# DanielLin94144/E2E-ASR-Pytorch

Hardware: AMD Instinct MI355X
Metric: audio frames/sec (fwd+bwd) LibriSpeech-100 joint CTC-att (higher is better)
Workload: dtype bf16; 1 GPU; config/librispeech_asr.yaml (vgg 0, 4xBiLSTM-320, joint CTC-att 0.5), B=16 x T=1200 x D=160 per GPU, L=180, delta+SpecAugment on GPU, fwd+losses+bwd+grad-allreduce+clip+Adadelta, dropout on; global_batch=16, frames_per_utt=1200, parallelism=dp1

## Files before the change

e2e-asr-pytorch_amd/csrc/ctc.hip:

```cpp
#include "common.h"

namespace {

struct CtcP {
    const float* lp;
    const int64_t* tgt;
    const int64_t* in_len;
    const int64_t* tgt_len;
    float* nll;
    float* loss;
    float* grad;
    float* alpha;
    float* beta;
    int B, T, V, L, Smax;
    float gscale;
};

__device__ __forceinline__ float lse2(float a, float b) {
    const float m = fmaxf(a, b);
    if (m == -INFINITY) return -INFINITY;
    return m + __logf(1.f + __expf(-fabsf(a - b)));
}

__device__ __forceinline__ float lse3(float a, float b, float c) {
    const float m = fmaxf(fmaxf(a, b), c);
    if (m == -INFINITY) return -INFINITY;
    const float md = __builtin_amdgcn_fmed3f(a, b, c), mn = fminf(fminf(a, b), c);
    return m + __logf(1.f + __expf(md - m) + __expf(mn - m));
}

constexpr int CTC_FCH = 8;
constexpr size_t CTC_GRAD_LDS = 60 * 1024;

__global__ __launch_bounds__(1024) void ctc_sweep_kernel(CtcP p, int CF) {
    extern __shared__ __attribute__((aligned(16))) unsigned char smem[];
    const int b = blockIdx.x, back = blockIdx.y;
    const int tid = threadIdx.x, NTH = blockDim.x;
    const int V = p.V, T = p.T;
    int tl = (int)p.tgt_len[b];
    tl = max(0, min(tl, p.L));
    const int S = 2 * tl + 1;
    int Tin = (int)p.in_len[b];
    Tin = max(0, min(Tin, T));
    int* ext = reinterpret_cast<int*>(smem);
    float* buf0 = reinterpret_cast<float*>(ext + p.Smax + 2) + 2;
    float* buf1 = buf0 + p.Smax + 6;
    float* s_lp = buf1 + p.Smax + 4;
    const float* lp = p.lp + (long)b * T * V;
    float* lat = (back ? p.beta : p.alpha) + (long)b * T * p.Smax;

    for (int s = tid; s < p.Smax + 2; s += NTH) ext[s] = (s < S && (s & 1)) ? (int)p.tgt[(long)b * p.L + (s >> 1)] : 0;
    for (int s = tid - 2; s < p.Smax + 2; s += NTH) { buf0[s] = -INFINITY; buf1[s] = -INFINITY; }
    __syncthreads();
    if (Tin == 0) {
        if (!back && tid == 0) {
            const float n = (tl == 0) ? 0.f : INFINITY;
            p.nll[b] = n;
        }
        return;
    }
// ... 16 lines not shown
        __syncthreads();
        for (int i = 0; i < nf; ++i) {
            const int t = back ? Tin - 1 - (c0 + i) : c0 + i;
            const float lpe = s_lp[(t - tlo) * V + e];
            float a;
            if (c0 + i == 0) {
                if (!back) a = (s == 0 || s == 1) ? lpe : -INFINITY;
                else       a = (s == S - 1 || s == S - 2) ? lpe : -INFINITY;
            } else {
                const int d1 = back ? 1 : -1;
                if (label) a = lse3(prev[sr], prev[sr + d1], skip ? prev[sr + 2 * d1] : -INFINITY);
                else       a = lse2(prev[sr], prev[sr + d1]);
                a += lpe;
            }
            if (sok) { cur[s] = a; lat[(long)t * p.Smax + s] = a; }
            __syncthreads();
            float* tmp = prev; prev = cur; cur = tmp;
        }
    }
    if (!back && tid == 0) {
        float ll = prev[S - 1];
        if (S > 1) ll = lse2(ll, prev[S - 2]);
        p.nll[b] = -ll;
    }
}

template <int FCH>
__global__ __launch_bounds__(1024) void ctc_grad_kernel(CtcP p) {
    extern __shared__ __attribute__((aligned(16))) unsigned char smem[];
    const int b = blockIdx.y, t0 = blockIdx.x * FCH;
    const int tid = threadIdx.x, NTH = blockDim.x, lane = tid & 63, wave = tid >> 6, nwave = NTH >> 6;
    const int V = p.V, T = p.T;
    int tl = (int)p.tgt_len[b];
    tl = max(0, min(tl, p.L));
    const int S = 2 * tl + 1;
    int Tin = (int)p.in_len[b];
    Tin = max(0, min(Tin, T));
    float* acc = reinterpret_cast<float*>(smem);
    float* blk = acc + FCH * V;
    const float* lp = p.lp + (long)b * T * V;
    float* grad = p.grad + (long)b * T * V;
    for (int i = tid; i < FCH * V; i += NTH) acc[i] = 0.f;
    const int s = tid;
    const bool sok = s < S;
    const int e = (sok && (s & 1)) ? (int)p.tgt[(long)b * p.L + (s >> 1)] : 0;
    const float nll = p.nll[b];
// ... 22 lines not shown
    for (int f = 0; f < FCH; ++f) {
        if (sok && (s & 1) && t0 + f < Tin) atomicAdd(&acc[f * V + e], occ[f]);
        const float bsum = wave_sum((sok && !(s & 1)) ? occ[f] : 0.f);
        if (lane == 0) blk[f * nwave + wave] = bsum;
    }
    __syncthreads();
    for (int i = tid; i < FCH * V; i += NTH) {
        const int f = i / V, v = i - f * V, t = t0 + f;
        if (t >= T) continue;
        float g = 0.f;
        if (t < Tin) {
            float a = acc[i];
            if (v == 0) for (int w = 0; w < nwave; ++w) a += blk[f * nwave + w];
            if (!(nll < INFINITY)) a = NAN;
            g = scale * (expf(lp[(long)t * V + v]) - a);
        }
        grad[(long)t * V + v] = g;
    }
}

}

extern "C" size_t asr_ctc_loss_workspace_bytes(int B, int T, int L) {
    return 2 * (size_t)B * T * (2 * (size_t)L + 1) * sizeof(float);
}

extern "C" int asr_ctc_loss(const float* logp, const int64_t* targets, const int64_t* input_len, const int64_t* target_len,
                            float* nll, float* loss, float* grad, int B, int T, int V, int L, float gscale,
                            void* workspace, size_t workspace_bytes, asr_stream_t stream) {
    ASR_REQUIRE(logp && targets && input_len && target_len && nll && loss && grad && workspace, ASR_E_ARG, "asr_ctc_loss: null pointer");
    ASR_REQUIRE(B > 0 && T > 0 && V > 1 && L > 0, ASR_E_ARG, "asr_ctc_loss: bad dims");
    ASR_REQUIRE(workspace_bytes >= asr_ctc_loss_workspace_bytes(B, T, L), ASR_E_ARG, "asr_ctc_loss: workspace too small");
    const int Smax = 2 * L + 1;
    float* wsf = (float*)workspace;
    CtcP p{logp, targets, input_len, target_len, nll, loss, grad, wsf, wsf + (size_t)B * T * Smax, B, T, V, L, Smax, gscale};
    ASR_REQUIRE(Smax <= 1024, ASR_E_UNSUPPORTED, "asr_ctc_loss: 2L+1=%d states exceed one workgroup", Smax);
    const int nthr = 64 * ((L + 1 + 63) / 64 + (L + 63) / 64);
    const size_t fixed = (size_t)(Smax + 2) * 4 + 2 * (size_t)(Smax + 6) * 4 + 16;
    int CF = (int)((60 * 1024 - fixed) / ((size_t)V * 4));
    ASR_REQUIRE(CF >= 1, ASR_E_UNSUPPORTED, "asr_ctc_loss: V=%d classes exceed the LDS budget: at most V=%d with 2L+1=%d states "
                "(one frame of log-probs beside the lattice buffers in 60 KB)", V, (int)((60 * 1024 - fixed) / 4), Smax);
    if (CF > T) CF = T;
    const size_t lds_s = fixed + (size_t)CF * V * 4;
    const size_t lds_g1 = (size_t)(V + nthr / 64) * 4;
    ASR_REQUIRE(lds_g1 <= CTC_GRAD_LDS, ASR_E_UNSUPPORTED, "asr_ctc_loss: V=%d classes exceed the %zu bytes of LDS of the gradient kernel",
                V, CTC_GRAD_LDS);
    int fch = CTC_FCH;
    while ((size_t)fch * lds_g1 > CTC_GRAD_LDS) fch >>= 1;
    hipStream_t st = (hipStream_t)stream;
    hipLaunchKernelGGL(ctc_sweep_kernel, dim3(B, 2), dim3(nthr), lds_s, st, p, CF);
    const dim3 gg(cdiv(T, fch), B);
    switch (fch) {
        case 8: hipLaunchKernelGGL(ctc_grad_kernel<8>, gg, dim3(nthr), 8 * lds_g1, st, p); break;
        case 4: hipLaunchKernelGGL(ctc_grad_kernel<4>, gg, dim3(nthr), 4 * lds_g1, st, p); break;
        case 2: hipLaunchKernelGGL(ctc_grad_kernel<2>, gg, dim3(nthr), 2 * lds_g1, st, p); break;
        default: hipLaunchKernelGGL(ctc_grad_kernel<1>, gg, dim3(nthr), lds_g1, st, p); break;
    }
    ASR_LAUNCH_CHECK("asr_ctc_loss");
    return ASR_OK;
}
```

e2e-asr-pytorch_amd/csrc/decoder_persist.hip:

```cpp
#include "decoder_plan.h"

static int g_persist_fwd = -1, g_persist_bwd = -1;
static int g_stream_fwd = -1, g_stream_bwd = -1;
extern "C" int asr_att_decoder_set_persistent(int flags) {
    const int old = (g_persist_fwd != 0 ? 1 : 0) | (g_persist_bwd != 0 ? 2 : 0) | (g_stream_fwd > 0 ? 4 : 0) | (g_stream_bwd > 0 ? 8 : 0);
    g_persist_fwd = flags & 1; g_persist_bwd = (flags >> 1) & 1; g_stream_fwd = (flags >> 2) & 1; g_stream_bwd = (flags >> 3) & 1;
    return old;
}
static void read_switches() {
    if (g_persist_fwd < 0) g_persist_fwd = env_switch("ASR_DEC_PERSIST", 1);
    if (g_persist_bwd < 0) g_persist_bwd = env_switch("ASR_DEC_PERSIST_BWD", 1);
    if (g_stream_fwd < 0) g_stream_fwd = env_switch("ASR_DEC_STREAM", 0);
    if (g_stream_bwd < 0) g_stream_bwd = env_switch("ASR_DEC_STREAM", 0);
}
static FwdPlan fwd_plan(const asr_dec_dims_t& d) { read_switches(); return chosen_plan(persist_plan(d), stream_plan_f(d), g_stream_fwd); }
static BwdPlan bwd_plan(const asr_dec_dims_t& d) { read_switches(); return chosen_plan(persist_plan_b(d), stream_plan_b(d), g_stream_bwd); }

DecPlanInfo dec_fwd_plan_info(const asr_dec_dims_t& d) {
    read_switches();
    const FwdPlan r = persist_plan(d), s = stream_plan_f(d);
    return {chosen_plan(r, s, g_stream_fwd).kind, 0, 0, std::max(r.total, s.total)};
}
DecPlanInfo dec_bwd_plan_info(const asr_dec_dims_t& d) {
    read_switches();
    const BwdPlan r = persist_plan_b(d), s = stream_plan_b(d), pl = chosen_plan(r, s, g_stream_bwd);
    return {pl.kind, pl.NT, std::max(r.NT, s.NT), std::max(r.total, s.total)};
}
float* dec_bwd_dgates(const asr_dec_dims_t& d, void* work) { return bwd_work(d, bwd_plan(d), work).dgates; }

namespace {

size_t dec_fwd_persist_lds(int TE, int NT, int A, int E, int Ks, int KCP, int UPW, int SG2) {
    const int EPL = 16 * cdiv(TE, 16);
    const ConvGeo cg = conv_geo(EPL, Ks);
    const size_t shorts = (size_t)((TE * A + 7) & ~7)
                        + ((TE * E + 7) & ~7)
                        + EPL * FCVX_LD
                        + 8 * cg.IMG_LD
                        + 32 * cg.WKP;
    const size_t floats = (size_t)2 * KCP
                        + ((A + 3) & ~3)
                        + ((A + 3) & ~3)
                        + ((NT * TE + 2 * Ks + 8 + 3) & ~3)
                        + NCW * EPL
                        + ((4 * UPW + 3) & ~3)
                        + (size_t)NT * 2 * SG2;
    return 2 * shorts + 4 * floats;
}

// ... 948 lines not shown
```

e2e-asr-pytorch_amd/src/asr.py:

```python
import math

import torch
import torch.nn as nn

from src import functions as F_hip
from src import hipabi as H
from src.module import RNNLayer, Downsampler, LocationAwareAttention, LSTMParams
from src.util import init_weights_, init_gate_

ALIGN = 64


class _RunCtx(object):

    def __init__(self, model):
        self.anchor = model._anchor
        self.prec = model.prec
        self._model = model

    def next_seed(self):
        self._model._drop_counter += 1
        return (self._model.seed * 1000003 + self._model._drop_counter) & 0xFFFFFFFFFFFF


# ... 210 lines not shown
        msg = ['Model spec.| Encoder\'s downsampling rate of time axis is {}.'.format(self.encoder.sample_rate)]
        if self.encoder.vgg == 1:
            msg.append('           | VGG Extractor w/ time downsampling rate = 4 in encoder enabled.')
        if self.encoder.vgg == 5:
            msg.append('           | VGG Extractor w/ Layer normalization and downsampling rate = 4.')
        if self.enable_ctc:
            msg.append('           | CTC training on encoder enabled ( lambda = {}).'.format(self.ctc_weight))
        if self.enable_att:
            msg.append('           | {} attention decoder enabled ( lambda = {}).'.format(self.attention.mode, 1 - self.ctc_weight))
        msg.append('           | HIP path (gfx950), contraction precision = {}.'.format('bf16' if self.prec == H.BF16 else 'fp32'))
        return msg

    def forward(self, audio_feature, feature_len, decode_step, tf_rate=0.0, teacher=None,
                emb_decoder=None, get_dec_state=False, get_logit=False, ctc_async=False):
        if not audio_feature.is_cuda:
            raise RuntimeError('ASR (HIP path) needs CUDA tensors; there is no CPU fallback')
        if emb_decoder is not None:
            raise NotImplementedError('embedding-regulariser plugin is outside the HIP path')
        ctx = _RunCtx(self)
        feature_len = feature_len.to(audio_feature.device)
        ctc_output, att_output, att_seq, dec_state = None, None, None, None
        encode_feature, encode_len = self.encoder(audio_feature.float(), feature_len, ctx)
        encode_feature = F_hip.to_f32_fn(encode_feature)
        side_ctc = (self.enable_ctc and self.enable_att and self.training and torch.is_grad_enabled() and H.overlap_enabled()
                    and H.ctc_side_enabled() and getattr(self, '_dp', None) is None)
        if self.enable_ctc:
            self.ctc_layer[0]._asr_defer = getattr(self, '_dp', None) is None or H.overlap_dp_enabled()
            if side_ctc:
                with H.side_branch(True, encode_feature, encode_len):
                    ctc_output = F_hip.CTCHeadFn.apply(ctx.anchor, encode_feature, self.ctc_layer[0], self.prec, get_logit)
                ctc_output._asr_side = bool(ctc_async)
            else:
                ctc_output = F_hip.CTCHeadFn.apply(ctx.anchor, encode_feature, self.ctc_layer[0], self.prec, get_logit)
        if self.enable_att:
            L = int(decode_step)
            if not (self.decoder.fast and self.attention.fast and self.emb_drop == 0.0):
                from src.variants import variant_decoder
                att_output, att_seq, hs = variant_decoder(self, ctx.anchor, encode_feature, encode_len, L, teacher,
                                                          float(tf_rate) if teacher is not None else 1.0, ctx)
                if get_dec_state:
                    dec_state = hs
                if side_ctc and not ctc_async:
                    H.join_branch(ctc_output)
                return ctc_output, encode_len, att_output, att_seq, dec_state
            att_output, att_seq, hs = F_hip.AttDecoderFn.apply(ctx.anchor, encode_feature, encode_len, teacher, L, self, self.prec,
                                                               float(tf_rate) if teacher is not None else 1.0)
            if get_dec_state:
                dec_state = hs[:, :, -1, :]
        if side_ctc and not ctc_async:
            H.join_branch(ctc_output)
        return ctc_output, encode_len, att_output, att_seq, dec_state

    def fix_ctc_layer(self):
        for param in self.ctc_layer.parameters():
# ... 2 lines not shown
```

e2e-asr-pytorch_amd/src/functions.py:

```python
import contextlib
import ctypes
import weakref

import torch

from src import hipabi as H


def _empty(shape, like):
    return torch.empty(shape, dtype=torch.float32, device=like.device)


def out_frames(layer, T):
    r = layer.sample_rate
    if r == 1:
        return T, 1
    return ((T + r - 1) // r, 1) if layer.sample_style == 'drop' else (T // r, r)


def lstm_rec(layer, gates, B, T, prec, dy=None, c=None):
    Hd, ND = layer.dim, layer.nd
    nbytes = H.lib().asr_lstm_workspace_bytes(B, Hd, ND)
    ws = H.handoff_acquire(nbytes, gates.device)
    tail = (B, T, Hd, ND, prec, H.ptr(ws), nbytes, H.stream_ptr())
# ... 413 lines not shown
            H.call('asr_loss_mix', H.ptr(g), H.ptr(sv[1]), None, None, H.ptr(gb), H.stream_ptr())
        return ga, None, gb, None


class CTCLossFn(torch.autograd.Function):
    @staticmethod
    def forward(ctx, logp_btv, targets, input_len, target_len):
        logp = logp_btv.contiguous()
        B, T, V = logp.shape
        targets = targets.contiguous()
        L = targets.shape[1]
        if 2 * L + 1 > 1024:
            L = max(1, int(target_len.max()))
            targets = targets[:, :L].contiguous()
        dev = logp.device
        nll = torch.empty(B, dtype=torch.float32, device=dev)
        loss = torch.empty((), dtype=torch.float32, device=dev)
        grad = _empty((B, T, V), logp)
        nbytes = H.lib().asr_ctc_loss_workspace_bytes(B, T, L)
        ws = torch.empty(nbytes, dtype=torch.uint8, device=dev)
        targets = targets.to(dev, torch.int64)
        il = input_len.to(dev, torch.int64).contiguous()
        tl = target_len.to(dev, torch.int64).contiguous()
        H.call('asr_ctc_loss', H.ptr(logp), H.ptr(targets), H.ptr(il), H.ptr(tl), H.ptr(nll), H.ptr(loss), H.ptr(grad),
               B, T, V, L, 1.0, H.ptr(ws), nbytes, H.stream_ptr())
        ctx.save_for_backward(grad)
        ctx.nll = nll
        return loss

    @staticmethod
    def backward(ctx, gout):
        (grad,) = ctx.saved_tensors
        return scale_by_device_scalar(grad, gout), None, None, None


class SeqLossFn(torch.autograd.Function):
    @staticmethod
    def forward(ctx, logits_rv, target_r, mode, classes, smoothing):
        logits = logits_rv.contiguous()
        R, V = logits.shape
        tgt = target_r.to(logits_rv.device, torch.int64).contiguous()
        dev = logits.device
        dl = _empty((R, V), logits)
        loss = torch.empty((), dtype=torch.float32, device=dev)
        acc = torch.empty(4, dtype=torch.float32, device=dev)
        H.call('asr_xent', H.ptr(logits), H.ptr(tgt), R, H.ptr(dl), H.ptr(loss), H.ptr(acc), 1, R, V, mode, classes,
               smoothing, 1.0, H.stream_ptr())
        ctx.save_for_backward(dl)
# ... 233 lines not shown
```

e2e-asr-pytorch_amd/src/hipabi.py:

```python
import atexit
import ctypes
import os

import torch

_HERE = os.path.dirname(os.path.abspath(__file__))
LIB_PATH = os.environ.get('ASR_HIP_LIB') or os.path.join(os.path.dirname(_HERE), 'lib', 'libasr_hip.so')

F32, BF16 = 0, 1
DEBUG_KEEP = os.environ.get('ASR_DEBUG_KEEP', '0') == '1'
ACT_NONE, ACT_TANH, ACT_RELU = 0, 1, 2
MAX_DEC_LAYERS = 4

_vp, _i, _l, _f, _u64, _sz = ctypes.c_void_p, ctypes.c_int, ctypes.c_long, ctypes.c_float, ctypes.c_uint64, ctypes.c_size_t


class DecDims(ctypes.Structure):
    _fields_ = [(n, _i) for n in ('B', 'Tp', 'E', 'A', 'Q', 'Dd', 'NL', 'V', 'Kn', 'Ks', 'L')] + [('temperature', _f)]


_DEC_W_FIELDS = ['Wq', 'bq', 'Wk', 'bk', 'Wconv', 'Wproj', 'wg', 'bg', 'emb']


class DecWeights(ctypes.Structure):
    _fields_ = [(n, _vp) for n in _DEC_W_FIELDS] + \
               [(n, _vp * MAX_DEC_LAYERS) for n in ('Wih', 'Whh', 'bih', 'bhh')] + [('Wc', _vp), ('bc', _vp)]


class DecState(ctypes.Structure):
    _fields_ = ([(n, _vp) for n in ('key', 'att', 'q', 'xin', 'gates', 'cs', 'hs', 'logits', 'energy', 'conv', 'key16', 'enc16', 'work')]
                + [('work_bytes', ctypes.c_size_t), ('tokens', _vp)])


class BeamStep(ctypes.Structure):
    _fields_ = ([(n, _vp) for n in ('att_logp', 'lm_logp', 'psi', 'candidates', 'alive_in', 'sum_in', 'ctcp_in', 'len_in', 'seq_in', 'score_in',
                                    'alive_out', 'sum_out', 'ctcp_out', 'len_out', 'seq_out', 'score_out', 'last_token', 'parent', 'ctc_index',
                                    'tokens')]
                + [('tokens_ld', _l)]
                + [(n, _vp) for n in ('min_len', 'max_len', 'done', 'fin_n', 'fin_len', 'fin_avg', 'fin_seq', 'fin_score')]
                + [(n, _i) for n in ('U', 'beam', 'V', 'C', 'Lmax', 't')]
                + [(n, _f) for n in ('ctc_weight', 'lm_weight', 'eos_threshold')])


ATT_DOT, ATT_LOC = 0, 1
BEAM_ATTEND_MAX_ROWS, BEAM_ATTEND_MAX_T = 16, 8192
CTC_BEAM_MAX = 16


class BeamAttend(ctypes.Structure):
    _fields_ = ([(n, _vp) for n in ('key', 'value', 'q', 'loc', 'wg', 'bg', 'enc_len', 'attn')] + [('attn_ld', _l), ('ctx', _vp)]
                + [(n, _l) for n in ('ctx_ld', 'ld_k', 'ld_v', 'ld_l')]
                + [(n, _i) for n in ('U', 'rows_per_utt', 'NH', 'NHv', 'Tp', 'A', 'Dv', 'mode', 'kv_bf16')] + [('temperature', _f)])


_P = ctypes.POINTER

SIGNATURES = {
    'asr_gemm': [_vp, _vp, _vp, _vp, _i, _i, _i, _l, _l, _l, _i, _i, _i, _i, _i, _i, _l, _l, _l, _i, _i, _i, _vp],
    'asr_lstm_fwd': [_vp, _vp, _vp, _vp, _vp, _i, _i, _i, _i, _i, _vp, _sz, _vp],
    'asr_lstm_bwd': [_vp, _vp, _vp, _vp, _i, _i, _i, _i, _i, _vp, _sz, _vp],
    'asr_dropout_downsample_fwd': [_vp, _vp, _i, _i, _i, _i, _i, _i, _f, _u64, _vp],
    'asr_dropout_downsample_bwd': [_vp, _vp, _i, _i, _i, _i, _i, _i, _f, _u64, _vp],
    'asr_dropout_mask': [_vp, _l, _f, _u64, _vp],
    'asr_act_bwd': [_vp, _vp, _vp, _l, _i, _vp],
    'asr_colsum': [_vp, _l, _i, _i, _vp, _vp],
    'asr_colsum2': [_vp, _l, _i, _i, _vp, _vp, _vp],
    'asr_log_softmax': [_vp, _vp, _l, _i, _vp],
    'asr_logsoftmax_relu_bwd': [_vp, _vp, _vp, _vp, _l, _i, _vp],
    'asr_layernorm_fwd': [_vp, _vp, _vp, _vp, _vp, _l, _i, _f, _i, _vp],
    'asr_layernorm_bwd': [_vp, _vp, _vp, _vp, _vp, _vp, _vp, _vp, _l, _i, _i, _vp],
    'asr_ctc_loss': [_vp, _vp, _vp, _vp, _vp, _vp, _vp, _i, _i, _i, _i, _f, _vp, _sz, _vp],
    'asr_xent': [_vp, _vp, _l, _vp, _vp, _vp, _i, _i, _i, _i, _i, _f, _f, _vp],
    'asr_att_decoder_fwd': [_P(DecDims), _P(DecWeights), _vp, _vp, _vp, _i, _P(DecState), _i, _vp],
    'asr_att_decoder_bwd': [_P(DecDims), _P(DecWeights), _P(DecWeights), _vp, _vp, _P(DecState), _vp, _vp, _vp, _sz, _i, _vp],
    'asr_att_decoder_bwd_ex': [_P(DecDims), _P(DecWeights), _P(DecWeights), _vp, _vp, _P(DecState), _vp, _vp, _vp, _sz, _i, _i,
                               ctypes.POINTER(_i), _vp],
    'asr_att_decoder_bwd_params': [_P(DecDims), _P(DecWeights), _P(DecWeights), _vp, _vp, _P(DecState), _vp, _vp, _sz, _i, _i, _vp],
    'asr_fbank': [_vp, _vp, _vp, _vp, _vp, _vp, _i, _i, _i, _i, _i, _i, _i, _f, _f, _f, _vp, _sz, _vp],
    'asr_delta_stack': [_vp, _vp, _vp, _vp, _i, _i, _i, _i, _i, _vp],
    'asr_specaug': [_vp, _vp, _vp, _vp, _i, _i, _i, _i, _i, _u64, _vp],
    'asr_specaug_ws': [_vp, _vp, _vp, _vp, _i, _i, _i, _i, _i, _u64, _vp, _sz, _vp],
    'asr_conv3x3': [_vp, _vp, _vp, _vp, _i, _i, _i, _i, _i, _i, _i, _i, _i, _vp],
    'asr_conv_weight_permute': [_vp, _vp, _i, _i, _i, _vp],
    'asr_vgg16_im2col': [_vp, _vp, _i, _i, _i, _i, _i, _vp],
    'asr_conv_weight_pack16': [_vp, _vp, _i, _i, _i, _i, _vp],
    'asr_conv_weight_fold': [_vp, _vp, _i, _i, _i, _vp],
    'asr_conv3x3_16': [_vp, _vp, _vp, _vp, _i, _i, _i, _i, _i, _i, _i, _i, _i, _vp],
    'asr_conv3x3_16_wgrad': [_vp, _vp, _vp, _i, _i, _i, _i, _i, _i, _i, _vp],
    'asr_maxpool2x2_16_fwd': [_vp, _vp, _vp, _i, _i, _i, _i, _i, _i, _vp],
    'asr_maxpool2x2_16_bwd': [_vp, _vp, _vp, _i, _i, _i, _i, _i, _i, _vp],
    'asr_ln_freq16_fwd': [_vp, _vp, _vp, _vp, _vp, _i, _i, _i, _i, _f, _i, _vp],
    'asr_ln_freq16_bwd': [_vp, _vp, _vp, _vp, _vp, _vp, _vp, _vp, _vp, _i, _i, _i, _i, _i, _vp],
    'asr_vgg16_output': [_vp, _vp, _i, _i, _i, _i, _vp],
    'asr_vgg16_output_bwd': [_vp, _vp, _i, _i, _i, _i, _vp],
# ... 47 lines not shown
    'asr_cast_bf16': [_vp, _vp, _l, _vp],
    'asr_cast_f32': [_vp, _vp, _l, _i, _vp],
    'asr_rnn_pack_weights': [_vp, _vp, _vp, _vp, _vp, _vp, _vp, _vp, _vp, _i, _i, _i, _i, _vp],
    'asr_dropout_downsample16_fwd': [_vp, _l, _l, _vp, _i, _i, _i, _i, _i, _i, _f, _u64, _vp],
    'asr_dropout_downsample16_bwd': [_vp, _vp, _i, _i, _i, _i, _i, _i, _f, _u64, _vp],
    'asr_act_bwd16': [_vp, _vp, _vp, _l, _i, _vp],
    'asr_colsum16': [_vp, _l, _i, _i, _vp, _vp, _i, _vp],
    'asr_debug_occupy': [_i, _i, ctypes.c_double, _vp],
    'asr_scrub_workspace': [_vp, _sz, _vp, _vp],
    'asr_stream_create_cu_mask': [_i, _i, ctypes.POINTER(_vp)],
    'asr_stream_destroy': [_vp],
}
_RESTYPES = {
    'asr_last_error': (ctypes.c_char_p, []),
    'asr_device_arch': (ctypes.c_char_p, []),
    'asr_version': (ctypes.c_int, []),
    'asr_lstm_workspace_bytes': (_sz, [_i, _i, _i]),
    'asr_gru_rec_workspace_bytes': (_sz, [_i, _i]),
    'asr_specaug_workspace_bytes': (_sz, [_i]),
    'asr_lstm_set_persistent': (ctypes.c_int, [_i]),
    'asr_lstm_plan': (ctypes.c_int, [_i, _i, _i, _i, _i]),
    'asr_lstm16_workspace_bytes': (_sz, [_i, _i, _i, _i]),
    'asr_ctc_loss_workspace_bytes': (_sz, [_i, _i, _i]),
    'asr_ctc_beam_search_workspace_bytes': (_sz, [_i, _i, _i]),
    'asr_ctc_align_workspace_bytes': (_sz, [_i, _i, _i]),
    'asr_fbank_workspace_bytes': (_sz, [_i, _i, _i, _i]),
    'asr_att_decoder_bwd_workspace_bytes': (_sz, [_P(DecDims)]),
    'asr_att_decoder_fwd_work_bytes': (_sz, [_P(DecDims)]),
    'asr_att_decoder_set_persistent': (ctypes.c_int, [_i]),
    'asr_att_decoder_bwd_status_offset': (_sz, [_P(DecDims)]),
    'asr_att_decoder_bwd_persistent_tiles': (ctypes.c_int, [_P(DecDims)]),
    'asr_att_decoder_fwd_plan': (ctypes.c_int, [_P(DecDims)]),
    'asr_att_decoder_bwd_plan': (ctypes.c_int, [_P(DecDims)]),
    'asr_beam_attend_resident_max_t': (ctypes.c_int, [_i]),
}


class HipLibraryMissing(RuntimeError):
    pass


def _load():
    if not os.path.exists(LIB_PATH):
        raise HipLibraryMissing(
            'libasr_hip.so not found at %s — build it with `python -c "import __graft_entry__ as g; g.build()"` '
            '(there is no CPU fallback for the HIP path)' % LIB_PATH)
    lib = ctypes.CDLL(LIB_PATH)
    for name, argtypes in SIGNATURES.items():
        fn = getattr(lib, name)
        fn.argtypes = argtypes
        fn.restype = ctypes.c_int
    for name, (rt, at) in _RESTYPES.items():
        fn = getattr(lib, name)
        fn.argtypes = at
        fn.restype = rt
    return lib
# ... 121 lines not shown


def configure_rec_units(hidden_dims):
    global REC_UNITS
    if 'ASR_REC_UNITS' in os.environ or not hidden_dims:
        return REC_UNITS
    units = max(rec_units_for(h) for h in hidden_dims)
    if units != REC_UNITS:
        if _side['stream'] is not None or _masked:
            release_streams()
        REC_UNITS = units
    return REC_UNITS


def overlap_enabled():
    return os.environ.get('ASR_OVERLAP', '1') != '0'


def overlap_dp_enabled():
    return overlap_enabled() and os.environ.get('ASR_OVERLAP_DP', '0') == '1'


def ctc_side_enabled():
    return os.environ.get('ASR_CTC_SIDE', '0') == '1'


_work = {}


def work_stream():
    dev = torch.cuda.current_device()
    if dev not in _work:
        _work[dev] = torch.cuda.Stream()
    return _work[dev]


def masked_stream(first, count):
    key = (torch.cuda.current_device(), first, count)
    if key not in _masked:
        out = _vp()
        call('asr_stream_create_cu_mask', first, count, ctypes.byref(out))
        _masked[key] = (torch.cuda.ExternalStream(out.value), out.value)
    return _masked[key][0]


def release_streams():
    if not _masked:
# ... 67 lines not shown


class side_branch:

    def __init__(self, wait, *tensors):
        self.wait, self.tensors = wait, [t for t in tensors if t is not None]

    def __enter__(self):
        if _side['stream'] is None:
            _side['stream'] = masked_stream(REC_UNITS, 32 - REC_UNITS) if overlap_enabled() else torch.cuda.Stream()
        side = _side['stream']
        if self.wait:
            side.wait_stream(torch.cuda.current_stream())
        _side['keep'].extend(self.tensors)
        self.ctx = torch.cuda.stream(side)
        self.ctx.__enter__()
        return side

    def __exit__(self, *exc):
        _side['pending'] = True
        return self.ctx.__exit__(*exc)


def join_branch(*tensors):
    cur = torch.cuda.current_stream()
    if _side['stream'] is not None:
        cur.wait_stream(_side['stream'])
    _side['keep'].extend(t for t in tensors if t is not None)


def defer_side(fn, *tensors):
    ev = torch.cuda.Event()
    ev.record(torch.cuda.current_stream())
    _side['deferred'].append((fn, ev, tensors))
    _side['pending'] = True
    if not _side.get('callback'):
        try:
            torch.autograd.Variable._execution_engine.queue_callback(join_side)
            _side['callback'] = True
        except RuntimeError:
            pass


def begin_forward():
    if _side['deferred'] or _side.get('callback'):
        _side['deferred'] = []
        _side['callback'] = False
        del _side['keep'][:]


def flush_side(after=None):
    todo, _side['deferred'] = _side['deferred'], []
    for fn, ev, tensors in todo:
        with on_side_stream(ev, *tensors) as side:
            if after is not None:
                side.wait_event(after)
            fn()


def join_side():
    todo, _side['deferred'] = _side['deferred'], []
    cur = torch.cuda.current_stream()
    for fn, ev, tensors in todo:
        cur.wait_event(ev)
        fn()
    if _side['stream'] is not None and _side['pending']:
        torch.cuda.current_stream().wait_stream(_side['stream'])
    _side['pending'] = False
    _side['callback'] = False
    del _side['keep'][:]
# ... 93 lines not shown
```

e2e-asr-pytorch_amd/src/step.py:

```python
import torch


def train_step(model, optimizer, ctc_crit, att_crit, feat, feat_len, txt, decode_step, tf_rate=1.0, dp=None,
               clip=5.0, txt_len=None, optimize=True):
    from src import hipabi as H
    cur = torch.cuda.current_stream()
    if not (feat.is_cuda and H.overlap_enabled() and (dp is None or H.overlap_dp_enabled())) or cur != torch.cuda.default_stream():
        return _train_step(model, optimizer, ctc_crit, att_crit, feat, feat_len, txt, decode_step, tf_rate, dp, clip, txt_len, optimize)
    work = H.work_stream()
    work.wait_stream(cur)
    with torch.cuda.stream(work):
        out = _train_step(model, optimizer, ctc_crit, att_crit, feat, feat_len, txt, decode_step, tf_rate, dp, clip, txt_len, optimize)
    cur.wait_stream(work)
    for v in out.values():
        if torch.is_tensor(v):
            v.record_stream(cur)
    return out


def scale_weight(w_dev, k):
    from src import hipabi as H
    from src.functions import loss_weight
    if not torch.is_tensor(w_dev):
        return loss_weight(float(w_dev) * k, torch.device('cuda', torch.cuda.current_device()))
    w = w_dev.reshape(1).to(torch.float32).contiguous()
    out = torch.empty(1, dtype=torch.float32, device=w.device)
    H.call('asr_loss_mix', H.ptr(w), H.ptr(loss_weight(k, w.device)), None, None, H.ptr(out), H.stream_ptr())
    return out


def _train_step(model, optimizer, ctc_crit, att_crit, feat, feat_len, txt, decode_step, tf_rate=1.0, dp=None,
                clip=5.0, txt_len=None, optimize=True):
    from src import hipabi as H
    opt = optimizer.opt if hasattr(optimizer, 'opt') else optimizer
    opt.zero_grad()
    if txt_len is None:
        txt_len = torch.sum(txt != 0, dim=-1)
    ctc_output, encode_len, att_output, att_align, _ = model(feat, feat_len, decode_step, tf_rate=tf_rate, teacher=txt, ctc_async=True)
    total, ctc_loss, att_loss = None, None, None
    from src.functions import LossMixFn, loss_weight
    dev = feat.device
    if ctc_output is not None:
        if getattr(ctc_output, '_asr_side', False):
            with H.side_branch(False, txt, txt_len):
                ctc_loss = ctc_crit(ctc_output.transpose(0, 1), txt, encode_len, txt_len)
            H.join_branch(ctc_loss, ctc_output)
        else:
            ctc_loss = ctc_crit(ctc_output.transpose(0, 1), txt, encode_len, txt_len)
    w_att = None
    if att_output is not None:
        b, t, _ = att_output.shape
        att_loss = att_crit(att_output.view(b * t, -1), txt[:, :t].reshape(-1))
        if dp is not None and dp.world > 1:
            w_att = scale_weight(dp.ce_weight(txt_len.sum()), 1 - model.ctc_weight)
        else:
            w_att = loss_weight(1 - model.ctc_weight, dev)
    if ctc_loss is not None and att_loss is not None:
        total = LossMixFn.apply(ctc_loss, loss_weight(model.ctc_weight, dev), att_loss, w_att)
    elif ctc_loss is not None:
        total = LossMixFn.apply(ctc_loss, loss_weight(model.ctc_weight, dev), None, None)
    else:
        total = LossMixFn.apply(att_loss, w_att, None, None)
    total.backward()
    H.join_side()
    grad_mul = 1.0
    if dp is not None:
        dp.finish()
        grad_mul = dp.grad_mul
    normsq = opt.grad_norm()
    if optimize:
        opt.step(clip=clip, grad_mul=grad_mul, use_norm=True)
    return {'total_loss': total.detach(), 'ctc_loss': ctc_loss, 'att_loss': att_loss, 'grad_normsq': normsq,
            'grad_mul': grad_mul, 'ctc_output': ctc_output, 'att_output': att_output, 'att_align': att_align,
            'encode_len': encode_len}
```

include/asr_hip.h:

```cpp
#ifndef ASR_HIP_H
#define ASR_HIP_H
#include <stdint.h>
#include <stddef.h>

#ifdef __cplusplus
extern "C" {
#endif

#define ASR_OK 0
#define ASR_E_ARG (-1)
#define ASR_E_LAUNCH (-2)
#define ASR_E_UNSUPPORTED (-3)

#define ASR_F32 0
#define ASR_BF16 1

#define ASR_ACT_NONE 0
#define ASR_ACT_TANH 1
#define ASR_ACT_RELU 2

typedef void* asr_stream_t;

const char* asr_last_error(void);
int asr_version(void);
// ... 43 lines not shown

int asr_ragged_align(const void* src, void* dst, const int64_t* lens, int B, int T, int ND, int W, int elem_bytes,
                     asr_stream_t stream);
int asr_ragged_unalign(const void* src, long src_bstride, long src_off, void* dst, const int64_t* lens, int B, int T,
                       int ND, int H, int T2, int rate, int style, int elem_bytes, asr_stream_t stream);
int asr_ragged_zero_tail(void* buf, const int64_t* lens, int B, int T, int Ttot, int t_off, int W, int elem_bytes,
                         asr_stream_t stream);

int asr_act_bwd(const float* dout, const float* out, float* dpre, long n, int act, asr_stream_t stream);
int asr_colsum(const float* A, long lda, int M, int N, float* out, asr_stream_t stream);
int asr_colsum2(const float* A, long lda, int M, int N, float* out, float* out2, asr_stream_t stream);
int asr_log_softmax(const float* x, float* out, long rows, int V, asr_stream_t stream);
int asr_logsoftmax_relu_bwd(const float* dlogp, const float* logp, const float* act, float* dpre,
                            long rows, int V, asr_stream_t stream);
int asr_layernorm_fwd(const float* x, const float* w, const float* b, float* y, float* stats,
                      long rows, int n, float eps, int relu, asr_stream_t stream);
int asr_layernorm_bwd(const float* dy, const float* x, const float* w, const float* b, const float* stats,
                      float* dx, float* dw, float* db, long rows, int n, int relu, asr_stream_t stream);

size_t asr_ctc_loss_workspace_bytes(int B, int T, int L);
int asr_ctc_loss(const float* logp, const int64_t* targets, const int64_t* input_len, const int64_t* target_len,
                 float* nll, float* loss, float* grad, int B, int T, int V, int L, float gscale,
                 void* workspace, size_t workspace_bytes, asr_stream_t stream);

int asr_xent(const float* logits, const int64_t* targets, long target_ld, float* dlogits, float* loss,
             float* accum2, int B, int L, int V, int mode, int classes, float smoothing, float gscale,
             asr_stream_t stream);

#define ASR_MAX_DEC_LAYERS 4
typedef struct {
    int B, Tp, E;
    int A, Q;
    int Dd, NL, V;
    int Kn, Ks;
    int L;
    float temperature;
} asr_dec_dims_t;

typedef struct {
    const float *Wq, *bq;
    const float *Wk, *bk;
    const float *Wconv;
    const float *Wproj;
    const float *wg, *bg;
    const float *emb;
    const float *Wih[ASR_MAX_DEC_LAYERS], *Whh[ASR_MAX_DEC_LAYERS];
// ... 11 lines not shown
    float* key;
    float* att;
    float* q;
    float* xin;
    float* gates;
    float* cs;
    float* hs;
    float* logits;
    float* energy;
    float* conv;
    void* key16;
    void* enc16;
    void* work;
    size_t work_bytes;
    int64_t* tokens;
} asr_dec_state_t;

int asr_att_decoder_fwd(const asr_dec_dims_t* dims, const asr_dec_weights_t* weights,
                        const float* enc, const int64_t* enc_len, const int64_t* teacher, int teacher_ld,
                        const asr_dec_state_t* state, int prec, asr_stream_t stream);
size_t asr_att_decoder_bwd_workspace_bytes(const asr_dec_dims_t* dims);
int asr_att_decoder_set_persistent(int flags);
int asr_att_decoder_fwd_plan(const asr_dec_dims_t* dims);
int asr_att_decoder_bwd_plan(const asr_dec_dims_t* dims);
int asr_att_decoder_bwd_persistent_tiles(const asr_dec_dims_t* dims);
size_t asr_att_decoder_bwd_status_offset(const asr_dec_dims_t* dims);
size_t asr_att_decoder_fwd_work_bytes(const asr_dec_dims_t* dims);
int asr_att_decoder_bwd(const asr_dec_dims_t* dims, const asr_dec_weights_t* weights, const asr_dec_grads_t* grads,
                        const float* enc, const int64_t* enc_len, const asr_dec_state_t* state,
                        const float* dlogits, float* denc,
                        void* workspace, size_t workspace_bytes, int prec, asr_stream_t stream);

int asr_att_decoder_bwd_ex(const asr_dec_dims_t* dims, const asr_dec_weights_t* weights, const asr_dec_grads_t* grads,
                           const float* enc, const int64_t* enc_len, const asr_dec_state_t* state,
                           const float* dlogits, float* denc,
                           void* workspace, size_t workspace_bytes, int prec, int defer_params, int* looped_out,
                           asr_stream_t stream);
int asr_att_decoder_bwd_params(const asr_dec_dims_t* dims, const asr_dec_weights_t* weights, const asr_dec_grads_t* grads,
                               const float* enc, const int64_t* enc_len, const asr_dec_state_t* state, const float* dlogits,
                               void* workspace, size_t workspace_bytes, int looped, int prec, asr_stream_t stream);

int asr_sumsq(const float* x, long n, double* out, asr_stream_t stream);
int asr_scale(float* x, long n, float k, asr_stream_t stream);
int asr_scale_dev(const float* in, float* out, long n, const float* alpha, asr_stream_t stream);
int asr_loss_mix(const float* a, const float* wa, const float* b, const float* wb, float* out, asr_stream_t stream);
int asr_status_collect(const void* const* abort_words, int n, unsigned* status, asr_stream_t stream);
// ... 150 lines not shown
```

Baseline: 1.138 million frames/s.

## Run CTC loss on a side stream beside the persistent decoder by default

Turns on the side-stream CTC branch by default. It adds a merged CTC sweep kernel that runs the forward and backward sweeps in one workgroup, claims utterances through global atomics and steers them by XCD. The merged kernel and the gradient kernel pad their LDS request so they can only fit on CUs that the persistent attention decoder leaves free, which lets CTC overlap the decoder without taking its resources. In exchange it adds a header memset, atomic work-claiming, an extra stream wait, and a new path that depends on the fit conditions.

Measured after the change: 1.145 million frames/s (median of 6 runs). About the same (+0.5%).

```diff
diff --git a/e2e-asr-pytorch_amd/csrc/ctc.hip b/e2e-asr-pytorch_amd/csrc/ctc.hip
--- a/e2e-asr-pytorch_amd/csrc/ctc.hip
+++ b/e2e-asr-pytorch_amd/csrc/ctc.hip
@@ -1,4 +1,5 @@
 #include "common.h"
+#include <algorithm>
 
 namespace {
 
@@ -32,10 +33,8 @@
 constexpr int CTC_FCH = 8;
 constexpr size_t CTC_GRAD_LDS = 60 * 1024;
 
-__global__ __launch_bounds__(1024) void ctc_sweep_kernel(CtcP p, int CF) {
-    extern __shared__ __attribute__((aligned(16))) unsigned char smem[];
-    const int b = blockIdx.x, back = blockIdx.y;
-    const int tid = threadIdx.x, NTH = blockDim.x;
+__device__ __forceinline__ void ctc_sweep_utt(const CtcP& p, const int CF, const int b, const int back, const int tid, const int NTH,
+                                              unsigned char* smem) {
     const int V = p.V, T = p.T;
     int tl = (int)p.tgt_len[b];
     tl = max(0, min(tl, p.L));
@@ -98,6 +97,61 @@
         float ll = prev[S - 1];
         if (S > 1) ll = lse2(ll, prev[S - 2]);
         p.nll[b] = -ll;
+    }
+}
+
+__global__ __launch_bounds__(1024) void ctc_sweep_kernel(CtcP p, int CF) {
+    extern __shared__ __attribute__((aligned(16))) unsigned char smem[];
+    ctc_sweep_utt(p, CF, blockIdx.x, blockIdx.y, threadIdx.x, blockDim.x, smem);
+}
+
+constexpr int CTC_W_XCD = 0;
+constexpr int CTC_W_NEXT = 8;
+constexpr int CTC_W_ARRIVED = 9;
+constexpr int CTC_W_UTT = 16;
+inline size_t ctc_hdr_bytes(int B) { return (size_t)(CTC_W_UTT + 2 * B) * sizeof(unsigned); }
+
+__global__ __launch_bounds__(1024) void ctc_sweep_merged_kernel(CtcP p, int CF, unsigned* hdr, int half_bytes) {
+    extern __shared__ __attribute__((aligned(16))) unsigned char smem[];
+    __shared__ int s_b, s_stay;
+    const int NTH = blockDim.x >> 1;
+    const int back = (int)threadIdx.x >= NTH ? 1 : 0;
+    const int tid = threadIdx.x - back * NTH;
+    unsigned char* mine = smem + (size_t)back * half_bytes;
+    unsigned* claim = hdr + CTC_W_UTT;
+    unsigned* done = claim + p.B;
+    if (threadIdx.x == 0) {
+        const unsigned xcc = __builtin_amdgcn_s_getreg((3 << 11) | 20) & 7u;
+        const unsigned ticket = __hip_atomic_fetch_add(&hdr[CTC_W_XCD + xcc], 1u, __ATOMIC_RELAXED, __HIP_MEMORY_SCOPE_AGENT);
+        int b = -1;
+        const unsigned cand = xcc + 8u * ticket;
+        if (ticket < (unsigned)((p.B + 7) >> 3) && cand < (unsigned)p.B &&
+            __hip_atomic_exchange(&claim[cand], 1u, __ATOMIC_RELAXED, __HIP_MEMORY_SCOPE_AGENT) == 0u) b = (int)cand;
+        const unsigned arrived = __hip_atomic_fetch_add(&hdr[CTC_W_ARRIVED], 1u, __ATOMIC_ACQ_REL, __HIP_MEMORY_SCOPE_AGENT);
+        s_b = b;
+        s_stay = (b >= 0 || arrived + 1u == gridDim.x) ? 1 : 0;
+    }
+    __syncthreads();
+    if (!s_stay) return;
+    int b = s_b;
+    while (true) {
+        if (b >= 0) {
+            ctc_sweep_utt(p, CF, b, back, tid, NTH, mine);
+            if (threadIdx.x == 0) __hip_atomic_fetch_add(&done[b], 1u, __ATOMIC_RELAXED, __HIP_MEMORY_SCOPE_AGENT);
+        }
+        __syncthreads();
+        if (threadIdx.x == 0) {
+            int nb = -1;
+            while (true) {
+                const unsigned n = __hip_atomic_fetch_add(&hdr[CTC_W_NEXT], 1u, __ATOMIC_RELAXED, __HIP_MEMORY_SCOPE_AGENT);
+                if (n >= (unsigned)p.B) break;
+                if (__hip_atomic_exchange(&claim[n], 1u, __ATOMIC_RELAXED, __HIP_MEMORY_SCOPE_AGENT) == 0u) { nb = (int)n; break; }
+            }
+            s_b = nb;
+        }
+        __syncthreads();
+        b = s_b;
+        if (b < 0) return;
     }
 }
 
@@ -166,12 +220,28 @@
 }
 
 extern "C" size_t asr_ctc_loss_workspace_bytes(int B, int T, int L) {
-    return 2 * (size_t)B * T * (2 * (size_t)L + 1) * sizeof(float);
+    return 2 * (size_t)B * T * (2 * (size_t)L + 1) * sizeof(float) + ctc_hdr_bytes(B);
+}
+
+static int ctc_sweep_threads(int L) { return 64 * ((L + 1 + 63) / 64 + (L + 63) / 64); }
+
+extern "C" int asr_ctc_loss_merged_threads(int L) {
+    if (L < 1) return 0;
+    const int n = 2 * ctc_sweep_threads(L);
+    return n <= 1024 ? n : 0;
 }
 
 extern "C" int asr_ctc_loss(const float* logp, const int64_t* targets, const int64_t* input_len, const int64_t* target_len,
                             float* nll, float* loss, float* grad, int B, int T, int V, int L, float gscale,
                             void* workspace, size_t workspace_bytes, asr_stream_t stream) {
+    return asr_ctc_loss_ex(logp, targets, input_len, target_len, nll, loss, grad, B, T, V, L, gscale, workspace, workspace_bytes,
+                           ASR_CTC_SPLIT, 0, stream);
+}
+
+extern "C" int asr_ctc_loss_ex(const float* logp, const int64_t* targets, const int64_t* input_len, const int64_t* target_len,
+                               float* nll, float* loss, float* grad, int B, int T, int V, int L, float gscale,
+                               void* workspace, size_t workspace_bytes, int form, size_t min_lds, asr_stream_t stream) {
+    ASR_REQUIRE(form == ASR_CTC_SPLIT || form == ASR_CTC_MERGED || form == ASR_CTC_MERGED_MIN_GRID, ASR_E_ARG, "asr_ctc_loss: form %d", form);
     ASR_REQUIRE(logp && targets && input_len && target_len && nll && loss && grad && workspace, ASR_E_ARG, "asr_ctc_loss: null pointer");
     ASR_REQUIRE(B > 0 && T > 0 && V > 1 && L > 0, ASR_E_ARG, "asr_ctc_loss: bad dims");
     ASR_REQUIRE(workspace_bytes >= asr_ctc_loss_workspace_bytes(B, T, L), ASR_E_ARG, "asr_ctc_loss: workspace too small");
@@ -179,7 +249,7 @@
     float* wsf = (float*)workspace;
     CtcP p{logp, targets, input_len, target_len, nll, loss, grad, wsf, wsf + (size_t)B * T * Smax, B, T, V, L, Smax, gscale};
     ASR_REQUIRE(Smax <= 1024, ASR_E_UNSUPPORTED, "asr_ctc_loss: 2L+1=%d states exceed one workgroup", Smax);
-    const int nthr = 64 * ((L + 1 + 63) / 64 + (L + 63) / 64);
+    const int nthr = ctc_sweep_threads(L);
     const size_t fixed = (size_t)(Smax + 2) * 4 + 2 * (size_t)(Smax + 6) * 4 + 16;
     int CF = (int)((60 * 1024 - fixed) / ((size_t)V * 4));
     ASR_REQUIRE(CF >= 1, ASR_E_UNSUPPORTED, "asr_ctc_loss: V=%d classes exceed the LDS budget: at most V=%d with 2L+1=%d states "
@@ -192,13 +262,32 @@
     int fch = CTC_FCH;
     while ((size_t)fch * lds_g1 > CTC_GRAD_LDS) fch >>= 1;
     hipStream_t st = (hipStream_t)stream;
-    hipLaunchKernelGGL(ctc_sweep_kernel, dim3(B, 2), dim3(nthr), lds_s, st, p, CF);
+    if (form != ASR_CTC_SPLIT && asr_ctc_loss_merged_threads(L)) {
+        constexpr size_t LDS_CAP = 160 * 1024 - 2048;
+        const size_t half = (lds_s + 15) & ~(size_t)15;
+        const size_t lds_m = std::max(2 * half, min_lds);
+        ASR_REQUIRE(lds_m <= LDS_CAP, ASR_E_UNSUPPORTED, "asr_ctc_loss: the merged sweep would need %zu bytes of LDS (limit %zu)", lds_m, LDS_CAP);
+        static unsigned char attr_[32];
+        if (first_on_device(attr_)) hipFuncSetAttribute((const void*)ctc_sweep_merged_kernel, hipFuncAttributeMaxDynamicSharedMemorySize, (int)LDS_CAP);
+        unsigned* hdr = (unsigned*)(wsf + 2 * (size_t)B * T * Smax);
+        hipMemsetAsync(hdr, 0, ctc_hdr_bytes(B), st);
+        const int grid = form == ASR_CTC_MERGED_MIN_GRID ? 1 : 8 * (cdiv(B, 8) + 6);
+        hipLaunchKernelGGL(ctc_sweep_merged_kernel, dim3(grid), dim3(2 * nthr), lds_m, st, p, CF, hdr, (int)half);
+    } else {
+        ASR_REQUIRE(min_lds == 0, ASR_E_UNSUPPORTED, "asr_ctc_loss: L=%d has no merged sweep to run beside other workgroups", L);
+        hipLaunchKernelGGL(ctc_sweep_kernel, dim3(B, 2), dim3(nthr), lds_s, st, p, CF);
+    }
     const dim3 gg(cdiv(T, fch), B);
+    auto launch_grad = [&](auto kernel, int frames) {
+        const size_t lds_g = std::max((size_t)frames * lds_g1, min_lds);
+        if (lds_g > 64 * 1024) hipFuncSetAttribute((const void*)kernel, hipFuncAttributeMaxDynamicSharedMemorySize, (int)(160 * 1024 - 2048));
+        hipLaunchKernelGGL(kernel, gg, dim3(nthr), lds_g, st, p);
+    };
     switch (fch) {
-        case 8: hipLaunchKernelGGL(ctc_grad_kernel<8>, gg, dim3(nthr), 8 * lds_g1, st, p); break;
-        case 4: hipLaunchKernelGGL(ctc_grad_kernel<4>, gg, dim3(nthr), 4 * lds_g1, st, p); break;
-        case 2: hipLaunchKernelGGL(ctc_grad_kernel<2>, gg, dim3(nthr), 2 * lds_g1, st, p); break;
-        default: hipLaunchKernelGGL(ctc_grad_kernel<1>, gg, dim3(nthr), lds_g1, st, p); break;
+        case 8: launch_grad(ctc_grad_kernel<8>, 8); break;
+        case 4: launch_grad(ctc_grad_kernel<4>, 4); break;
+        case 2: launch_grad(ctc_grad_kernel<2>, 2); break;
+        default: launch_grad(ctc_grad_kernel<1>, 1); break;
     }
     ASR_LAUNCH_CHECK("asr_ctc_loss");
     return ASR_OK;
diff --git a/e2e-asr-pytorch_amd/csrc/decoder_persist.hip b/e2e-asr-pytorch_amd/csrc/decoder_persist.hip
--- a/e2e-asr-pytorch_amd/csrc/decoder_persist.hip
+++ b/e2e-asr-pytorch_amd/csrc/decoder_persist.hip
@@ -25,6 +25,16 @@
     read_switches();
     const BwdPlan r = persist_plan_b(d), s = stream_plan_b(d), pl = chosen_plan(r, s, g_stream_bwd);
     return {pl.kind, pl.NT, std::max(r.NT, s.NT), std::max(r.total, s.total)};
+}
+extern "C" size_t asr_att_decoder_ctc_side_lds(const asr_dec_dims_t* dims) {
+    if (!dims) return 0;
+    read_switches();
+    if (!g_persist_fwd) return 0;
+    const FwdPlan pl = fwd_plan(*dims);
+    const int cpx = cdiv(dims->B, 8);
+    if (pl.kind != 1 || dims->B > 16 || 32 - cpx * pl.NT < cpx) return 0;
+    const size_t cu_lds = 160 * 1024, need = cu_lds - std::min(cu_lds, pl.lds) + 2048;
+    return need <= cu_lds - 2048 ? need : 0;
 }
 float* dec_bwd_dgates(const asr_dec_dims_t& d, void* work) { return bwd_work(d, bwd_plan(d), work).dgates; }
 
diff --git a/e2e-asr-pytorch_amd/src/asr.py b/e2e-asr-pytorch_amd/src/asr.py
--- a/e2e-asr-pytorch_amd/src/asr.py
+++ b/e2e-asr-pytorch_amd/src/asr.py
@@ -256,14 +256,20 @@
         ctc_output, att_output, att_seq, dec_state = None, None, None, None
         encode_feature, encode_len = self.encoder(audio_feature.float(), feature_len, ctx)
         encode_feature = F_hip.to_f32_fn(encode_feature)
-        side_ctc = (self.enable_ctc and self.enable_att and self.training and torch.is_grad_enabled() and H.overlap_enabled()
-                    and H.ctc_side_enabled() and getattr(self, '_dp', None) is None)
+        side_lds = 0
+        if (ctc_async and self.enable_ctc and self.enable_att and self.training and torch.is_grad_enabled() and H.overlap_enabled()
+                and getattr(self, '_dp', None) is None and self.prec == H.BF16 and teacher is not None and float(tf_rate) == 1.0
+                and self.decoder.fast and self.attention.fast and self.emb_drop == 0.0):
+            side_lds = H.ctc_side_plan(F_hip._dec_dims(self, encode_feature.shape[0], encode_feature.shape[1], int(decode_step)),
+                                       teacher.shape[1])
+        side_ctc = side_lds > 0
+        self.ctc_side_taken = side_ctc
         if self.enable_ctc:
             self.ctc_layer[0]._asr_defer = getattr(self, '_dp', None) is None or H.overlap_dp_enabled()
             if side_ctc:
                 with H.side_branch(True, encode_feature, encode_len):
                     ctc_output = F_hip.CTCHeadFn.apply(ctx.anchor, encode_feature, self.ctc_layer[0], self.prec, get_logit)
-                ctc_output._asr_side = bool(ctc_async)
+                ctc_output._asr_side = side_lds
             else:
                 ctc_output = F_hip.CTCHeadFn.apply(ctx.anchor, encode_feature, self.ctc_layer[0], self.prec, get_logit)
         if self.enable_att:
diff --git a/e2e-asr-pytorch_amd/src/functions.py b/e2e-asr-pytorch_amd/src/functions.py
--- a/e2e-asr-pytorch_amd/src/functions.py
+++ b/e2e-asr-pytorch_amd/src/functions.py
@@ -459,8 +459,9 @@
         targets = targets.to(dev, torch.int64)
         il = input_len.to(dev, torch.int64).contiguous()
         tl = target_len.to(dev, torch.int64).contiguous()
-        H.call('asr_ctc_loss', H.ptr(logp), H.ptr(targets), H.ptr(il), H.ptr(tl), H.ptr(nll), H.ptr(loss), H.ptr(grad),
-               B, T, V, L, 1.0, H.ptr(ws), nbytes, H.stream_ptr())
+        form = H._ctc_form
+        H.call('asr_ctc_loss_ex', H.ptr(logp), H.ptr(targets), H.ptr(il), H.ptr(tl), H.ptr(nll), H.ptr(loss), H.ptr(grad),
+               B, T, V, L, 1.0, H.ptr(ws), nbytes, form['form'], form['min_lds'], H.stream_ptr())
         ctx.save_for_backward(grad)
         ctx.nll = nll
         return loss
diff --git a/e2e-asr-pytorch_amd/src/hipabi.py b/e2e-asr-pytorch_amd/src/hipabi.py
--- a/e2e-asr-pytorch_amd/src/hipabi.py
+++ b/e2e-asr-pytorch_amd/src/hipabi.py
@@ -44,6 +44,7 @@
 
 ATT_DOT, ATT_LOC = 0, 1
 BEAM_ATTEND_MAX_ROWS, BEAM_ATTEND_MAX_T = 16, 8192
+CTC_SPLIT, CTC_MERGED, CTC_MERGED_MIN_GRID = 0, 1, 2
 CTC_BEAM_MAX = 16
 
 
@@ -70,6 +71,7 @@
     'asr_layernorm_fwd': [_vp, _vp, _vp, _vp, _vp, _l, _i, _f, _i, _vp],
     'asr_layernorm_bwd': [_vp, _vp, _vp, _vp, _vp, _vp, _vp, _vp, _l, _i, _i, _vp],
     'asr_ctc_loss': [_vp, _vp, _vp, _vp, _vp, _vp, _vp, _i, _i, _i, _i, _f, _vp, _sz, _vp],
+    'asr_ctc_loss_ex': [_vp, _vp, _vp, _vp, _vp, _vp, _vp, _i, _i, _i, _i, _f, _vp, _sz, _i, _sz, _vp],
     'asr_xent': [_vp, _vp, _l, _vp, _vp, _vp, _i, _i, _i, _i, _i, _f, _f, _vp],
     'asr_att_decoder_fwd': [_P(DecDims), _P(DecWeights), _vp, _vp, _vp, _i, _P(DecState), _i, _vp],
     'asr_att_decoder_bwd': [_P(DecDims), _P(DecWeights), _P(DecWeights), _vp, _vp, _P(DecState), _vp, _vp, _vp, _sz, _i, _vp],
@@ -163,6 +165,7 @@
     'asr_lstm_plan': (ctypes.c_int, [_i, _i, _i, _i, _i]),
     'asr_lstm16_workspace_bytes': (_sz, [_i, _i, _i, _i]),
     'asr_ctc_loss_workspace_bytes': (_sz, [_i, _i, _i]),
+    'asr_ctc_loss_merged_threads': (ctypes.c_int, [_i]),
     'asr_ctc_beam_search_workspace_bytes': (_sz, [_i, _i, _i]),
     'asr_ctc_align_workspace_bytes': (_sz, [_i, _i, _i]),
     'asr_fbank_workspace_bytes': (_sz, [_i, _i, _i, _i]),
@@ -173,6 +176,7 @@
     'asr_att_decoder_bwd_persistent_tiles': (ctypes.c_int, [_P(DecDims)]),
     'asr_att_decoder_fwd_plan': (ctypes.c_int, [_P(DecDims)]),
     'asr_att_decoder_bwd_plan': (ctypes.c_int, [_P(DecDims)]),
+    'asr_att_decoder_ctc_side_lds': (_sz, [_P(DecDims)]),
     'asr_beam_attend_resident_max_t': (ctypes.c_int, [_i]),
 }
 
@@ -340,7 +344,13 @@
 
 
 def ctc_side_enabled():
-    return os.environ.get('ASR_CTC_SIDE', '0') == '1'
+    return os.environ.get('ASR_CTC_SIDE', '1') != '0'
+
+
+def ctc_side_plan(dims, L):
+    if not ctc_side_enabled() or _lib.asr_ctc_loss_merged_threads(int(L)) == 0:
+        return 0
+    return int(_lib.asr_att_decoder_ctc_side_lds(ctypes.byref(dims)))
 
 
 _work = {}
@@ -454,6 +464,23 @@
         return self.ctx.__exit__(*exc)
 
 
+_ctc_form = {'form': CTC_SPLIT, 'min_lds': 0}
+
+
+class ctc_form:
+
+    def __init__(self, form, min_lds=0):
+        self.new = {'form': int(form), 'min_lds': int(min_lds)}
+
+    def __enter__(self):
+        self.old = dict(_ctc_form)
+        _ctc_form.update(self.new)
+
+    def __exit__(self, *exc):
+        _ctc_form.update(self.old)
+        return False
+
+
 def join_branch(*tensors):
     cur = torch.cuda.current_stream()
     if _side['stream'] is not None:
@@ -478,6 +505,8 @@
     if _side['deferred'] or _side.get('callback'):
         _side['deferred'] = []
         _side['callback'] = False
+        if _side['stream'] is not None and _side['keep']:
+            torch.cuda.current_stream().wait_stream(_side['stream'])
         del _side['keep'][:]
 
 
diff --git a/e2e-asr-pytorch_amd/src/step.py b/e2e-asr-pytorch_amd/src/step.py
--- a/e2e-asr-pytorch_amd/src/step.py
+++ b/e2e-asr-pytorch_amd/src/step.py
@@ -41,8 +41,9 @@
     from src.functions import LossMixFn, loss_weight
     dev = feat.device
     if ctc_output is not None:
-        if getattr(ctc_output, '_asr_side', False):
-            with H.side_branch(False, txt, txt_len):
+        side_lds = getattr(ctc_output, '_asr_side', 0)
+        if side_lds:
+            with H.side_branch(False, txt, txt_len), H.ctc_form(H.CTC_MERGED, side_lds):
                 ctc_loss = ctc_crit(ctc_output.transpose(0, 1), txt, encode_len, txt_len)
             H.join_branch(ctc_loss, ctc_output)
         else:
@@ -72,4 +73,4 @@
         opt.step(clip=clip, grad_mul=grad_mul, use_norm=True)
     return {'total_loss': total.detach(), 'ctc_loss': ctc_loss, 'att_loss': att_loss, 'grad_normsq': normsq,
             'grad_mul': grad_mul, 'ctc_output': ctc_output, 'att_output': att_output, 'att_align': att_align,
-            'encode_len': encode_len}
+            'encode_len': encode_len, 'ctc_side': bool(getattr(model, 'ctc_side_taken', False))}
diff --git a/include/asr_hip.h b/include/asr_hip.h
--- a/include/asr_hip.h
+++ b/include/asr_hip.h
@@ -89,6 +89,11 @@
 int asr_ctc_loss(const float* logp, const int64_t* targets, const int64_t* input_len, const int64_t* target_len,
                  float* nll, float* loss, float* grad, int B, int T, int V, int L, float gscale,
                  void* workspace, size_t workspace_bytes, asr_stream_t stream);
+enum { ASR_CTC_SPLIT = 0, ASR_CTC_MERGED = 1, ASR_CTC_MERGED_MIN_GRID = 2 };
+int asr_ctc_loss_ex(const float* logp, const int64_t* targets, const int64_t* input_len, const int64_t* target_len,
+                    float* nll, float* loss, float* grad, int B, int T, int V, int L, float gscale,
+                    void* workspace, size_t workspace_bytes, int form, size_t min_lds, asr_stream_t stream);
+int asr_ctc_loss_merged_threads(int L);
 
 int asr_xent(const float* logits, const int64_t* targets, long target_ld, float* dlogits, float* loss,
              float* accum2, int B, int L, int V, int mode, int classes, float smoothing, float gscale,
@@ -146,6 +151,7 @@
 size_t asr_att_decoder_bwd_workspace_bytes(const asr_dec_dims_t* dims);
 int asr_att_decoder_set_persistent(int flags);
 int asr_att_decoder_fwd_plan(const asr_dec_dims_t* dims);
+size_t asr_att_decoder_ctc_side_lds(const asr_dec_dims_t* dims);
 int asr_att_decoder_bwd_plan(const asr_dec_dims_t* dims);
 int asr_att_decoder_bwd_persistent_tiles(const asr_dec_dims_t* dims);
 size_t asr_att_decoder_bwd_status_offset(const asr_dec_dims_t* dims);
```
